# xytpai/kfunca

Hardware: AMD Instinct MI355X
Metric: bf16 GEMM TFLOP/s + causal-attn fwd+bwd tokens/s (higher is better)
Workload: dtype bf16

## Files before the change

kfunca_amd/csrc/device/attention.hip:

```cpp
#include <math.h>
#include <stdlib.h>

#include <algorithm>
#include <type_traits>

#include "common.h"

namespace kf {

typedef __attribute__((ext_vector_type(8))) __bf16 bf16x8;
typedef __attribute__((ext_vector_type(8))) _Float16 f16x8;
typedef __attribute__((ext_vector_type(4))) short s16x4;
typedef __attribute__((ext_vector_type(8))) short s16x8;
typedef __attribute__((ext_vector_type(16))) float f32x16;
typedef __attribute__((ext_vector_type(4))) float f32x4;

struct AttnArgs {
    const char *q, *k, *v, *o, *d_o;
    char *out, *dq, *dk, *dv;
    float *lse;
    const float *lse_r;
    float *delta;
    float *nlse, *ndelta;
    int64_t B, H, Sq, Skv, D;
// ... 400 lines not shown
        const int64_t kv0 = (int64_t)t * ABK;
        TL_STAMP(6)
        asm volatile("s_waitcnt vmcnt(4)" ::: "memory");
        TL_STAMP(0)
        __builtin_amdgcn_s_barrier();
        asm volatile("" ::: "memory");
        TL_STAMP(1)
        stage(t + 2, smem + ((t + 2) % SRING) * FBUF);
        TL_STAMP(2)
        const char *cur = smem + (t % SRING) * FBUF;
        const bool skip = !active || kv0 > qw + 31 || KF_MUT(1, t == 1 && qblk == nxb - 1);
        const bool diag = kv0 + ABK - 1 > qw;
        if (late && pending) s_pv<BF, DB>(smem + ((t + SRING - 1) % SRING) * FBUF + FTILE, vo, pf, o);
        pending = false;
        TL_STAMP(5)
        if (!skip) {
            if (diag) s_qk_sm<BF, true, D>(cur, qf, ko, o, pf, m_i, l_i, c, kv0, m, hl, a.defer TL_ARGS);
            else s_qk_sm<BF, false, D>(cur, qf, ko, o, pf, m_i, l_i, c, kv0, m, hl, a.defer TL_ARGS);
            TL_STAMP(4)
            if (late) pending = true;
            else s_pv<BF, DB>(cur + FTILE, vo, pf, o);
            TL_STAMP(5)
        }
    }
#if defined(KF_ATTN_TIMELINE) && KF_ATTN_TIMELINE != 2
    if (lane == 0 && g_attn_tl) {
        unsigned long long *dst = g_attn_tl + ((size_t)blockIdx.x * 2 + (pass & 1)) * 64 + wid * 8;
        for (int i = 0; i < 7; ++i) dst[i] = tl_acc[i];
        dst[7] = (unsigned long long)nt;
    }
#endif
#ifdef KF_ATTN_TIMELINE
    const unsigned long long tl_loop1 = __builtin_amdgcn_s_memtime();
#endif
    if (late && pending) s_pv<BF, DB>(smem + ((nt + SRING - 1) % SRING) * FBUF + FTILE, vo, pf, o);
    asm volatile("s_waitcnt vmcnt(0)" ::: "memory");
    __syncthreads();
    if (active) {
        a_store_rows<BF, DB>(smem + wid * 32 * OPAD, a.out + a_head(a.lo, bh, a.H) + qw * a.lo.sr, o, 1.f / l_i, a.lo.sr);
        if (a.lse && hl == 0) a.lse[bh * a.Sq + m] = (m_i * c + __builtin_amdgcn_logf(l_i)) * kLn2;
    }
    if (a.persist) __syncthreads();
#if defined(KF_ATTN_TIMELINE) && KF_ATTN_TIMELINE == 2
    if (lane == 0 && g_attn_tl) {
        unsigned long long *dst = g_attn_tl + ((size_t)blockIdx.x * 2 + (pass & 1)) * 64 + wid * 8;
        const unsigned long long tl_end = __builtin_amdgcn_s_memtime();
        dst[0] = tl_loop0 - tl_pass0, dst[1] = tl_loop1 - tl_loop0, dst[2] = tl_end - tl_loop1;
        dst[3] = dst[4] = dst[5] = dst[6] = 0;
        dst[7] = (unsigned long long)nt;
    }
#endif
  }
}

#ifndef KF_FWD_W4_INC
#define KF_FWD_W4_INC "attn_fwd_w4.inc"
#endif
#include KF_FWD_W4_INC
template <bool BF, bool SQ, bool D64 = false>
__global__ __launch_bounds__(256) void attn_fwd_w4_kernel(const AttnArgs a) {
    static_assert(!(SQ && D64), "the scaled-query form exists for head size 128 only");
    extern __shared__ __attribute__((aligned(16))) char smem[];
    const int nxb = (int)((a.Sq + FQ - 1) / FQ);
    const int nwx = a.persist ? nxb / 2 : nxb;
    const unsigned lds = (unsigned)(uintptr_t)(const __attribute__((address_space(3))) char *)smem;
    const int wid = __builtin_amdgcn_readfirstlane(threadIdx.x >> 6);
    const int dbytes = D64 ? 128 : 256;
    const unsigned kvn = (unsigned)((a.Skv - 1) * a.lk.sr + dbytes);
    const float c = a.scale_log2e, defer = a.defer;
    const int qsr = (int)a.lq.sr, kvsr = (int)a.lk.sr, osr = (int)a.lo.sr;
#pragma nounroll
    for (unsigned vwg = blockIdx.x; vwg < a.nvwg; vwg += gridDim.x) {
    int xb0;
    int64_t bh;
    a_block_map(nwx, a.nbh, a.xcd_map, xb0, bh, vwg);
    const char *kp = a.k + a_head_kv(a.lk, bh, a.H, a.G), *vp = a.v + a_head_kv(a.lv, bh, a.H, a.G);
    const char *qh = a.q + a_head(a.lq, bh, a.H);
    char *oh = a.out + a_head(a.lo, bh, a.H);
#pragma nounroll
    for (int pass = 0; pass < (a.persist ? 2 : 1); ++pass) {
        const int xb = ((pass & 1) != (a.persist_rev != 0)) ? nxb - 1 - xb0 : xb0;
        const int qblk = nxb - 1 - xb;
        const int64_t q0 = (int64_t)qblk * FQ;
        const char *qp = qh + q0 * a.lq.sr;
        char *op = oh + q0 * a.lo.sr;
        float *lsep = a.lse ? a.lse + bh * a.Sq + q0 : nullptr;
        const int T = (int)((q0 + FQ) / ABK);
        const int64_t qrows = a.Sq - q0 < FQ ? a.Sq - q0 : FQ;
        const unsigned qn = (unsigned)((qrows - 1) * a.lq.sr + dbytes), on = (unsigned)((qrows - 1) * a.lo.sr + dbytes), lsen = (unsigned)(qrows * 4);
        int mut = -1;
#ifdef KF_MUTANT
        if (a.mutant == 1 && qblk == nxb - 1) mut = 1;
#endif
#ifdef KF_FWD_W4_STAMPS
        unsigned long long *dbg = a.dbg;
        const unsigned dbgoff = (vwg * 2 + pass) * 4 * 32;
#define KF_W4_EXTRA , [dbg] "s"(dbg), [dbgoff] "s"(dbgoff)
#else
#define KF_W4_EXTRA
#endif
#define KF_W4_OPERANDS                                                                                                              \
    [qp] "s"(qp), [kp] "s"(kp), [vp] "s"(vp), [op] "s"(op), [lsep] "s"(lsep), [qsr] "s"(qsr), [kvsr] "s"(kvsr), [osr] "s"(osr), [T] "s"(T), \
        [wid] "s"(wid), [c] "s"(c), [defer] "s"(defer), [lds] "s"(lds), [mut] "s"(mut), [kvn] "s"(kvn), [qn] "s"(qn), [on] "s"(on), [lsen] "s"(lsen) KF_W4_EXTRA
        if constexpr (D64 && BF) asm volatile(KF_FWD_W4_D64_ASM_BF16 : : KF_W4_OPERANDS : KF_FWD_W4_CLOBBERS);
        else if constexpr (D64) asm volatile(KF_FWD_W4_D64_ASM_F16 : : KF_W4_OPERANDS : KF_FWD_W4_CLOBBERS);
        else if constexpr (BF && SQ) asm volatile(KF_FWD_W4_ASM_BF16_SQ : : KF_W4_OPERANDS : KF_FWD_W4_CLOBBERS);
        else if constexpr (BF) asm volatile(KF_FWD_W4_ASM_BF16 : : KF_W4_OPERANDS : KF_FWD_W4_CLOBBERS);
        else if constexpr (SQ) asm volatile(KF_FWD_W4_ASM_F16_SQ : : KF_W4_OPERANDS : KF_FWD_W4_CLOBBERS);
        else asm volatile(KF_FWD_W4_ASM_F16 : : KF_W4_OPERANDS : KF_FWD_W4_CLOBBERS);
#undef KF_W4_OPERANDS
#undef KF_W4_EXTRA
    }
    }
}

template <bool BF, int R>
__global__ __launch_bounds__(256) void attn_delta_kernel(const char *o, const char *d_o, float *delta, int64_t nrows, const float *lse, float *nlse,
                                                         float *ndelta, float rscale, AttnArgs::Lay lo, AttnArgs::Lay ldo, int64_t S, int64_t H, int nparts, int64_t Sc) {
    const int64_t row0 = (int64_t)blockIdx.x * (16 * R) + (threadIdx.x >> 4);
    const int part = threadIdx.x & 15;
    uint4 a[R], b[R];
#pragma unroll
    for (int i = 0; i < R; ++i) {
        a[i] = b[i] = uint4{0, 0, 0, 0};
        const int64_t row = row0 + 16 * i;
        const int64_t bh = row / Sc, sq = row - bh * Sc;
        if (row < nrows && sq < S && part < nparts) {
            a[i] = *(const uint4 *)(o + a_head(lo, bh, H) + sq * lo.sr + part * 16);
            b[i] = *(const uint4 *)(d_o + a_head(ldo, bh, H) + sq * ldo.sr + part * 16);
        }
    }
#pragma unroll
    for (int i = 0; i < R; ++i) {
        const int64_t row = row0 + 16 * i;
        float acc = 0.f;
        const uint32_t aw[4] = {a[i].x, a[i].y, a[i].z, a[i].w}, bw[4] = {b[i].x, b[i].y, b[i].z, b[i].w};
#pragma unroll
        for (int j = 0; j < 4; ++j) {
            float a0, a1, b0, b1;
            if constexpr (BF) {
                a0 = __uint_as_float(aw[j] << 16); a1 = __uint_as_float(aw[j] & 0xffff0000u);
                b0 = __uint_as_float(bw[j] << 16); b1 = __uint_as_float(bw[j] & 0xffff0000u);
            } else {
                a0 = f16_to_f32(f16_t{(uint16_t)(aw[j] & 0xffff)}); a1 = f16_to_f32(f16_t{(uint16_t)(aw[j] >> 16)});
                b0 = f16_to_f32(f16_t{(uint16_t)(bw[j] & 0xffff)}); b1 = f16_to_f32(f16_t{(uint16_t)(bw[j] >> 16)});
            }
            acc += a0 * b0 + a1 * b1;
        }
        for (int msk = 8; msk > 0; msk >>= 1) acc += __shfl_xor(acc, msk, 64);
        if (row < nrows && part == 0) {
            const int64_t bh = row / Sc, sq = row - bh * Sc;
            if (sq < S) {
                delta[bh * S + sq] = acc;
                if (nlse) {
                    nlse[row] = -lse[bh * S + sq] * rscale;
                    ndelta[row] = -acc;
                }
            } else if (nlse) {
                nlse[row] = 0.f;
                ndelta[row] = 0.f;
            }
        }
    }
}

template <bool BF, bool MASK, int D>
__device__ __forceinline__ void q_tile(const char *buf, const char *doslab, const typename AFrag<BF>::type (&qf)[D / 16], const int (&ko)[D / 16],
                                       const int (&vo)[D / 32][2], f32x16 (&dq)[D / 32], float c, float lse2, float dlt, int64_t kv0, int64_t m, int hl) {
    using frag_t = typename AFrag<BF>::type;
    constexpr int DB = D / 32;
    const char *vt = buf + FTILE;
#pragma unroll
    for (int sub = 0; sub < 2; ++sub) {
        f32x16 s, dp;
#pragma unroll
        for (int e = 0; e < 16; ++e) { s[e] = 0.f; dp[e] = 0.f; }
#pragma unroll
        for (int kg = 0; kg < D / 64; ++kg) {
#pragma unroll
            for (int kk = 4 * kg; kk < 4 * kg + 4; ++kk) s = a_mfma<BF>(*(const frag_t *)(buf + sub * 32 * AROW + ko[kk]), qf[kk], s);
            __builtin_amdgcn_sched_barrier(0);
        }
#pragma unroll
        for (int kg = 0; kg < D / 64; ++kg) {
#pragma unroll
            for (int kk = 4 * kg; kk < 4 * kg + 4; ++kk)
                dp = a_mfma<BF>(*(const frag_t *)(vt + sub * 32 * AROW + ko[kk]), *(const frag_t *)(doslab + ko[kk]), dp);
            __builtin_amdgcn_sched_barrier(0);
        }
#pragma unroll
        for (int e = 0; e < 16; ++e) {
            float p = __builtin_amdgcn_exp2f(__builtin_fmaf(s[e], c, -lse2));
            if (MASK && kv0 + sub * 32 + a_row(e, hl) > m) p = 0.f;
            s[e] = p * (dp[e] - dlt);
        }
        TrN<DB> ta;
        if (sub == 0) tr4_issue<0>(buf, vo, ta); else tr4_issue<32 * AROW>(buf, vo, ta);
        tr4_wait1(ta);
        { const frag_t df = a_pack<BF>(s, 0);
#pragma unroll
          for (int d = 0; d < DB; ++d) dq[d] = a_mfma<BF>(tr4_frag<BF, DB>(ta, d), df, dq[d]); }
        __builtin_amdgcn_sched_barrier(0);
        if (sub == 0) tr4_issue<16 * AROW>(buf, vo, ta); else tr4_issue<48 * AROW>(buf, vo, ta);
        tr4_wait1(ta);
        { const frag_t df = a_pack<BF>(s, 1);
#pragma unroll
          for (int d = 0; d < DB; ++d) dq[d] = a_mfma<BF>(tr4_frag<BF, DB>(ta, d), df, dq[d]); }
        __builtin_amdgcn_sched_barrier(0);
    }
}

constexpr int QSLAB = 32 * AROW;
constexpr int QLDS = FRING * FBUF + 8 * QSLAB;

template <bool BF, int D>
__global__ __launch_bounds__(FNT, 2) void attn_bwd_dq_v2_kernel(const AttnArgs a) {
    using frag_t = typename AFrag<BF>::type;
    constexpr int KS = D / 16, DB = D / 32;
    extern __shared__ __attribute__((aligned(16))) char smem[];
    const int lane = threadIdx.x & 63, wid = threadIdx.x >> 6, xl = lane & 31, hl = lane >> 5;
    int xb0;
    int64_t bh;
    const int nxb = (int)((a.Sq + FQ - 1) / FQ);
    const int nwx = a.persist ? nxb / (2 * a.persist) : nxb;
    a_block_map(nwx, a.nbh, a.xcd_map, xb0, bh);
    const char *Kg = a.k + a_head_kv(a.lk, bh, a.H, a.G);
    const char *Vg = a.v + a_head_kv(a.lv, bh, a.H, a.G);
    char *doslab = smem + FRING * FBUF + wid * QSLAB;
    int ko[KS], vo[DB][2];
#pragma unroll
    for (int kk = 0; kk < KS; ++kk) ko[kk] = a_off(xl, kk * 2 + hl);
#pragma unroll
    for (int d = 0; d < DB; ++d) {
        vo[d][0] = a_tr_lane_off(d * 32, 0);
        vo[d][1] = a_tr_lane_off(d * 32, 1);
    }
    const float c = a.scale * kLog2e;
#pragma nounroll
  for (int pass = 0; pass < (a.persist ? 2 * a.persist : 1); ++pass) {
    const int xp = xb0 + (pass >> 1) * nwx;
    const int xb = ((pass & 1) != (a.persist_rev != 0)) ? nxb - 1 - xp : xp;
    const int qblk = nxb - 1 - xb;
    const int64_t q0 = (int64_t)qblk * FQ, qw = q0 + wid * 32, m = qw + xl;
    const bool active = qw < a.Sq;

    frag_t qf[KS];
    float lse2 = 0.f, dlt = 0.f;
    if (active) {
        const char *Qg = a.q + a_head(a.lq, bh, a.H) + m * a.lq.sr;
#pragma unroll
        for (int kk = 0; kk < KS; ++kk) qf[kk] = *(const frag_t *)(Qg + (kk * 16 + 8 * hl) * 2);
        const char *dOw = a.d_o + a_head(a.ldo, bh, a.H) + qw * a.ldo.sr;
#pragma unroll
        for (int i = 0; i < 8; ++i)
            if (D == AD || ((lane + 64 * i) & 15) < D / 8) a_lst(doslab, lane + 64 * i, a_gld(dOw, lane + 64 * i, a.ldo.sr));
        lse2 = a.lse_r[bh * a.Sq + m] * kLog2e;
        dlt = a.delta[bh * a.Sq + m];
    } else {
#pragma unroll
        for (int kk = 0; kk < KS; ++kk)
#pragma unroll
            for (int j = 0; j < 8; ++j) qf[kk][j] = 0;
    }
    f32x16 dq[DB];
#pragma unroll
    for (int d = 0; d < DB; ++d)
#pragma unroll
        for (int e = 0; e < 16; ++e) dq[d][e] = 0.f;

    const int64_t q_end = q0 + FQ < a.Sq ? q0 + FQ : a.Sq;
    const int64_t kv_end = a.Skv < q_end ? a.Skv : q_end;
    const int nt = (int)((kv_end + ABK - 1) / ABK);
    auto stage = [&](int tile, char *buf) {
        const int64_t kv = (int64_t)(tile < nt ? tile : nt - 1) * ABK;
        f_stage<D>(Kg + kv * a.lk.sr, Vg + kv * a.lv.sr, buf, a.lk.sr, a.lv.sr);
    };
    asm volatile("s_waitcnt vmcnt(0) lgkmcnt(0)" ::: "memory");
    stage(0, smem);
    stage(1, smem + FBUF);
    for (int t = 0; t < nt; ++t) {
        const int64_t kv0 = (int64_t)t * ABK;
        asm volatile("s_waitcnt vmcnt(4)" ::: "memory");
        __builtin_amdgcn_s_barrier();
        asm volatile("" ::: "memory");
        stage(t + 2, smem + ((t + 2) % FRING) * FBUF);
        const char *cur = smem + (t % FRING) * FBUF;
        const bool skip = !active || kv0 > qw + 31 || KF_MUT(4, t == 0 && qblk == nxb - 1);
        const bool diag = kv0 + ABK - 1 > qw;
        if (!skip) {
            if (diag) q_tile<BF, true, D>(cur, doslab, qf, ko, vo, dq, c, lse2, dlt, kv0, m, hl);
            else q_tile<BF, false, D>(cur, doslab, qf, ko, vo, dq, c, lse2, dlt, kv0, m, hl);
        }
    }
    asm volatile("s_waitcnt vmcnt(0)" ::: "memory");
    __syncthreads();
    if (active) a_store_rows<BF, DB>(smem + wid * 32 * OPAD, a.dq + a_head(a.ldq, bh, a.H) + qw * a.ldq.sr, dq, a.scale, a.ldq.sr);
    if (a.persist) __syncthreads();
  }
}

constexpr int DQ_RING = 3;
constexpr int DQ_SLAB = 2 * DS_TILE;
constexpr int DQ_LDS = DQ_RING * FTILE + 8 * DQ_RING * DQ_SLAB;

template <bool BF, int HF, int KS, int DB>
__device__ __forceinline__ void dq_step(const char *kt, const int (&vo)[DB][2], unsigned dsb, f32x16 (&dq)[DB]) {
    s16x4 blo, bhi;
    TrN<DB> ta;
    asm volatile("ds_read_b64_tr_b16 %0, %2 offset:%c3\n\tds_read_b64_tr_b16 %1, %2 offset:%c4"
                 : "=&v"(blo), "=&v"(bhi)
                 : "v"(dsb), "n"(HF * DS_TILE + KS * 512), "n"(HF * DS_TILE + KS * 512 + 256)
                 : "memory");
    tr4_issue<(32 * HF + 16 * KS) * AROW>(kt, vo, ta);
    asm volatile("s_waitcnt lgkmcnt(0)" : "+v"(blo), "+v"(bhi) : : "memory");
    tr4_wait1(ta);
    s16x8 r;
    r[0] = blo[0]; r[1] = blo[1]; r[2] = blo[2]; r[3] = blo[3];
    r[4] = bhi[0]; r[5] = bhi[1]; r[6] = bhi[2]; r[7] = bhi[3];
    const auto b = __builtin_bit_cast(typename AFrag<BF>::type, r);
#pragma unroll
    for (int d = 0; d < DB; ++d) dq[d] = a_mfma<BF>(tr4_frag<BF, DB>(ta, d), b, dq[d]);
}

template <bool BF, int D>
__global__ __launch_bounds__(FNT, 2) void attn_bwd_dq_ds_kernel(const AttnArgs a) {
    constexpr int DB = D / 32;
    extern __shared__ __attribute__((aligned(16))) char smem[];
    const int lane = threadIdx.x & 63, wid = __builtin_amdgcn_readfirstlane(threadIdx.x >> 6);
    int xb0;
    int64_t bh;
    const int nxb = (int)((a.Sq + FQ - 1) / FQ);
    const int nwx = a.persist ? nxb / (2 * a.persist) : nxb;
    a_block_map(nwx, a.nbh, a.xcd_map, xb0, bh);
    bh += a.bh0;
    const char *Kg = a.k + a_head_kv(a.lk, bh, a.H, a.G);
    char *slab = smem + DQ_RING * FTILE + wid * DQ_RING * DQ_SLAB;
    int vo[DB][2];
#pragma unroll
    for (int d = 0; d < DB; ++d) {
        vo[d][0] = a_tr_lane_off(d * 32, 0);
        vo[d][1] = a_tr_lane_off(d * 32, 1);
    }
    const int grp = lane >> 4, qq = (lane >> 2) & 3, pp = lane & 3, h = grp >> 1;
    const unsigned smem_u = (unsigned)(uintptr_t)(const __attribute__((address_space(3))) char *)smem;
    const int sp = grp & 1;
    const unsigned ds_rd = smem_u + (unsigned)(slab - smem) + sp * 1024 + 64 * ((2 * h + (qq >> 1)) ^ (2 * sp)) + 32 * (qq & 1) + 16 * (pp & 1) + 8 * (pp >> 1);
    int ds_src[2];
#pragma unroll
    for (int pc = 0; pc < 2; ++pc) ds_src[pc] = pc * 1024 + (((lane >> 2) ^ (2 * pc)) * 4 + (lane & 3)) * 16;
    const int krow = lane >> 4, kpos = lane & 15;
#pragma nounroll
  for (int pass = 0; pass < (a.persist ? 2 * a.persist : 1); ++pass) {
    const int xp = xb0 + (pass >> 1) * nwx;
    const int xb = ((pass & 1) != (a.persist_rev != 0)) ? nxb - 1 - xp : xp;
    const int qblk = nxb - 1 - xb;
    const int64_t q0 = (int64_t)qblk * FQ, qw = q0 + wid * 32;
    const bool active = qw < a.Sq;
    const int sl = (int)(qw >> 5);
    f32x16 dq[DB];
#pragma unroll
    for (int d = 0; d < DB; ++d)
#pragma unroll
        for (int e = 0; e < 16; ++e) dq[d][e] = 0.f;
    const int64_t q_end = q0 + FQ < a.Sq ? q0 + FQ : a.Sq;
    const int64_t kv_end = a.Skv < q_end ? a.Skv : q_end;
    const int nt = (int)((kv_end + ABK - 1) / ABK);
    const char *dsg = a.ds + ((bh - a.bh0) * a.ds_pair + ds_row_base(qblk, a.ds_nkb, a.ds_tri) + wid) * DS_TILE;
    const int kwb_last = (int)(a.ds_nkb * 8 - 1);
    const int slw = qblk * 8 + wid;
    auto stage = [&](int tile, int slot) {
        const int tl = tile < nt ? tile : nt - 1;
        const int kfirst = tl * ABK, klast = (int)a.Skv - 1 - kfirst;
        const char *kg = Kg + (int64_t)kfirst * a.lk.sr;
#pragma unroll
        for (int i = 0; i < 2; ++i) {
            const int row0 = (wid * 2 + i) * 4, row = row0 + krow;
            const int chunk = kpos ^ (((row & 3) << 2) | ((row >> 2) & 3));
            const int srow = row < klast ? row : klast;
            if (D == AD || chunk < D / 8)
                __builtin_amdgcn_global_load_lds((const __attribute__((address_space(1))) void *)(kg + (int64_t)srow * a.lk.sr + chunk * 16),
                                                 (__attribute__((address_space(3))) void *)(smem + slot * FTILE + row0 * AROW), 16, 0, 0);
        }
#pragma unroll
        for (int hf = 0; hf < 2; ++hf) {
            int kwb = 2 * tl + hf;
            kwb = kwb < kwb_last ? kwb : kwb_last;
            kwb = kwb <= slw ? kwb : (slw < kwb_last ? slw : kwb_last);
            const char *tg = dsg + (int64_t)kwb * 8 * DS_TILE;
#pragma unroll
            for (int pc = 0; pc < 2; ++pc)
                __builtin_amdgcn_global_load_lds((const __attribute__((address_space(1))) void *)(tg + ds_src[pc]),
                                                 (__attribute__((address_space(3))) void *)(slab + slot * DQ_SLAB + hf * DS_TILE + pc * 1024), 16, 0, 0);
        }
    };
    stage(0, 0);
    stage(1, 1);
    for (int t = 0; t < nt; ++t) {
        asm volatile("s_waitcnt vmcnt(6)" ::: "memory");
        __builtin_amdgcn_s_barrier();
        asm volatile("" ::: "memory");
        stage(t + 2, (t + 2) % DQ_RING);
        const char *kt = smem + (t % DQ_RING) * FTILE;
        const unsigned dsb = ds_rd + (unsigned)((t % DQ_RING) * DQ_SLAB);
        if (active && 2 * t <= sl && !KF_MUT(3, t == 0 && qblk == nxb - 1)) {
            dq_step<BF, 0, 0, DB>(kt, vo, dsb, dq);
            dq_step<BF, 0, 1, DB>(kt, vo, dsb, dq);
            if (2 * t + 1 <= sl) {
                dq_step<BF, 1, 0, DB>(kt, vo, dsb, dq);
                dq_step<BF, 1, 1, DB>(kt, vo, dsb, dq);
            }
        }
    }
    asm volatile("s_waitcnt vmcnt(0)" ::: "memory");
    __syncthreads();
    if (active) a_store_rows<BF, DB>(smem + wid * 32 * OPAD, a.dq + a_head(a.ldq, bh, a.H) + qw * a.ldq.sr, dq, a.scale, a.ldq.sr,
                                     (int)(a.Sq - qw < 32 ? a.Sq - qw : 32));
    if (a.persist) __syncthreads();
  }
}

constexpr int BQS = 32;

constexpr int K4B = 128;
constexpr int K4SL = 2 * BQS * AROW + 256;
constexpr int K4PAIR = 2 * K4SL;
constexpr int K4LDS = 4 * K4PAIR;
constexpr bool K4_SPREAD = true;
static_assert(K4LDS >= 4 * 32 * OPAD, "epilogue slabs must fit");

template <int OFF>
__device__ __forceinline__ void k4_rows4(unsigned e, unsigned o, s16x8 (&f)[4]) {
    asm volatile("ds_read_b128 %0, %4 offset:%c6\n\tds_read_b128 %1, %5 offset:%c6\n\t"
                 "ds_read_b128 %2, %4 offset:%c7\n\tds_read_b128 %3, %5 offset:%c7"
                 : "=&v"(f[0]), "=&v"(f[1]), "=&v"(f[2]), "=&v"(f[3])
                 : "v"(e), "v"(o), "n"(OFF), "n"(OFF + 512)
                 : "memory");
}
template <int OFF>
__device__ __forceinline__ void k4_rowc(unsigned lr, f32x4 (&c)[4]) {
    asm volatile("ds_read_b128 %0, %4 offset:%c5\n\tds_read_b128 %1, %4 offset:%c6\n\t"
                 "ds_read_b128 %2, %4 offset:%c7\n\tds_read_b128 %3, %4 offset:%c8"
                 : "=&a"(c[0]), "=&a"(c[1]), "=&a"(c[2]), "=&a"(c[3])
                 : "v"(lr), "n"(OFF), "n"(OFF + 32), "n"(OFF + 64), "n"(OFF + 96)
                 : "memory");
}
struct K4Tr { s16x4 lo[4], hi[4]; };
template <int OFF>
__device__ __forceinline__ void k4_tr4(unsigned t0, unsigned t1, K4Tr &t) {
    asm volatile("ds_read_b64_tr_b16 %0, %8 offset:%c10\n\tds_read_b64_tr_b16 %1, %9 offset:%c10\n\t"
                 "ds_read_b64_tr_b16 %2, %8 offset:%c11\n\tds_read_b64_tr_b16 %3, %9 offset:%c11\n\t"
                 "ds_read_b64_tr_b16 %4, %8 offset:%c12\n\tds_read_b64_tr_b16 %5, %9 offset:%c12\n\t"
                 "ds_read_b64_tr_b16 %6, %8 offset:%c13\n\tds_read_b64_tr_b16 %7, %9 offset:%c13"
                 : "=&v"(t.lo[0]), "=&v"(t.hi[0]), "=&v"(t.lo[1]), "=&v"(t.hi[1]), "=&v"(t.lo[2]), "=&v"(t.hi[2]), "=&v"(t.lo[3]), "=&v"(t.hi[3])
                 : "v"(t0), "v"(t1), "n"(OFF), "n"(OFF + 512), "n"(OFF + 1024), "n"(OFF + 1536)
                 : "memory");
}
template <int N>
__device__ __forceinline__ void k4_wait4(s16x8 (&f)[4]) {
    asm volatile("s_waitcnt lgkmcnt(%c4)" : "+v"(f[0]), "+v"(f[1]), "+v"(f[2]), "+v"(f[3]) : "n"(N) : "memory");
}
template <int N>
__device__ __forceinline__ void k4_wait4c(s16x8 (&f)[4], f32x4 (&c)[4]) {
    asm volatile("s_waitcnt lgkmcnt(%c8)"
                 : "+v"(f[0]), "+v"(f[1]), "+v"(f[2]), "+v"(f[3]), "+a"(c[0]), "+a"(c[1]), "+a"(c[2]), "+a"(c[3])
                 : "n"(N)
                 : "memory");
}
template <int N>
__device__ __forceinline__ void k4_wait_tr(K4Tr &a) {
    asm volatile("s_waitcnt lgkmcnt(%c8)"
                 : "+v"(a.lo[0]), "+v"(a.hi[0]), "+v"(a.lo[1]), "+v"(a.hi[1]), "+v"(a.lo[2]), "+v"(a.hi[2]), "+v"(a.lo[3]), "+v"(a.hi[3])
                 : "n"(N)
                 : "memory");
}
template <bool BF>
__device__ __forceinline__ typename AFrag<BF>::type k4_frag(const K4Tr &t, int d) {
    s16x8 r;
    r[0] = t.lo[d][0]; r[1] = t.lo[d][1]; r[2] = t.lo[d][2]; r[3] = t.lo[d][3];
    r[4] = t.hi[d][0]; r[5] = t.hi[d][1]; r[6] = t.hi[d][2]; r[7] = t.hi[d][3];
    return __builtin_bit_cast(typename AFrag<BF>::type, r);
}
__device__ __forceinline__ f32x16 k4_acc(const f32x4 (&c)[4]) {
    f32x16 r;
#pragma unroll
    for (int g = 0; g < 4; ++g)
#pragma unroll
        for (int j = 0; j < 4; ++j) r[4 * g + j] = c[g][j];
    return r;
}

template <int OFF>
__device__ __forceinline__ void k4_rows4a(unsigned e, unsigned o, s16x8 (&f)[4]) {
    asm volatile("ds_read_b128 %0, %4 offset:%c6\n\tds_read_b128 %1, %5 offset:%c6\n\t"
                 "ds_read_b128 %2, %4 offset:%c7\n\tds_read_b128 %3, %5 offset:%c7"
                 : "=&a"(f[0]), "=&a"(f[1]), "=&a"(f[2]), "=&a"(f[3])
                 : "v"(e), "v"(o), "n"(OFF), "n"(OFF + 512)
                 : "memory");
}
template <int OFF>
__device__ __forceinline__ void k4_rowcv(unsigned lr, f32x4 (&c)[4]) {
    asm volatile("ds_read_b128 %0, %4 offset:%c5\n\tds_read_b128 %1, %4 offset:%c6\n\t"
                 "ds_read_b128 %2, %4 offset:%c7\n\tds_read_b128 %3, %4 offset:%c8"
                 : "=&v"(c[0]), "=&v"(c[1]), "=&v"(c[2]), "=&v"(c[3])
                 : "v"(lr), "n"(OFF), "n"(OFF + 32), "n"(OFF + 64), "n"(OFF + 96)
                 : "memory");
}
template <int N>
__device__ __forceinline__ void k4_wait4a_cv(s16x8 (&f)[4], f32x4 (&c)[4]) {
    asm volatile("s_waitcnt lgkmcnt(%c8)"
                 : "+a"(f[0]), "+a"(f[1]), "+a"(f[2]), "+a"(f[3]), "+v"(c[0]), "+v"(c[1]), "+v"(c[2]), "+v"(c[3])
                 : "n"(N)
                 : "memory");
}
template <int N>
__device__ __forceinline__ void k4_wait4a(s16x8 (&f)[4]) {
    asm volatile("s_waitcnt lgkmcnt(%c4)" : "+a"(f[0]), "+a"(f[1]), "+a"(f[2]), "+a"(f[3]) : "n"(N) : "memory");
}
template <int N>
__device__ __forceinline__ void k4_wait4_cv(s16x8 (&f)[4], f32x4 (&c)[4]) {
    asm volatile("s_waitcnt lgkmcnt(%c8)"
                 : "+v"(f[0]), "+v"(f[1]), "+v"(f[2]), "+v"(f[3]), "+v"(c[0]), "+v"(c[1]), "+v"(c[2]), "+v"(c[3])
                 : "n"(N)
                 : "memory");
}
template <int OFF>
__device__ __forceinline__ void k4_row1(unsigned a, s16x8 &f) { asm volatile("ds_read_b128 %0, %1 offset:%c2" : "=&v"(f) : "v"(a), "n"(OFF) : "memory"); }
template <int OFF>
__device__ __forceinline__ void k4_row1a(unsigned a, s16x8 &f) { asm volatile("ds_read_b128 %0, %1 offset:%c2" : "=&a"(f) : "v"(a), "n"(OFF) : "memory"); }
template <int OFF>
__device__ __forceinline__ void k4_rowc1(unsigned lr, f32x4 &c) { asm volatile("ds_read_b128 %0, %1 offset:%c2" : "=&v"(c) : "v"(lr), "n"(OFF) : "memory"); }
template <int OFF>
__device__ __forceinline__ void k4_trp(unsigned t0, unsigned t1, s16x4 &lo, s16x4 &hi) {
    asm volatile("ds_read_b64_tr_b16 %0, %2 offset:%c4\n\tds_read_b64_tr_b16 %1, %3 offset:%c4" : "=&v"(lo), "=&v"(hi) : "v"(t0), "v"(t1), "n"(OFF) : "memory");
}
template <bool BF, bool AA>
__device__ __forceinline__ void k4_mfma_first(f32x16 &acc, s16x8 &a, const typename AFrag<BF>::type &b, f32x16 &c) {
    if constexpr (BF) {
        if constexpr (AA) asm volatile("s_nop 1\n\tv_mfma_f32_32x32x16_bf16 %0, %1, %3, %2" : "=&v"(acc), "+a"(a), "+v"(c) : "a"(b));
        else asm volatile("s_nop 1\n\tv_mfma_f32_32x32x16_bf16 %0, %1, %3, %2" : "=&v"(acc), "+v"(a), "+v"(c) : "a"(b));
    } else {
        if constexpr (AA) asm volatile("s_nop 1\n\tv_mfma_f32_32x32x16_f16 %0, %1, %3, %2" : "=&v"(acc), "+a"(a), "+v"(c) : "a"(b));
        else asm volatile("s_nop 1\n\tv_mfma_f32_32x32x16_f16 %0, %1, %3, %2" : "=&v"(acc), "+v"(a), "+v"(c) : "a"(b));
    }
}
template <bool BF, bool AA>
__device__ __forceinline__ void k4_mfma_acc(f32x16 &acc, s16x8 &a, const typename AFrag<BF>::type &b) {
    if constexpr (BF) {
        if constexpr (AA) asm volatile("v_mfma_f32_32x32x16_bf16 %0, %1, %2, %0" : "+v"(acc), "+a"(a) : "a"(b));
        else asm volatile("v_mfma_f32_32x32x16_bf16 %0, %1, %2, %0" : "+v"(acc), "+v"(a) : "a"(b));
    } else {
        if constexpr (AA) asm volatile("v_mfma_f32_32x32x16_f16 %0, %1, %2, %0" : "+v"(acc), "+a"(a) : "a"(b));
        else asm volatile("v_mfma_f32_32x32x16_f16 %0, %1, %2, %0" : "+v"(acc), "+v"(a) : "a"(b));
    }
}
template <bool BF>
__device__ __forceinline__ void k4_mfma_first_t(f32x16 &acc, s16x8 &a, const typename AFrag<BF>::type &b, f32x16 &c, f32x16 &tag) {
    if constexpr (BF) asm volatile("s_nop 1\n\tv_mfma_f32_32x32x16_bf16 %0, %1, %4, %2\n\ts_nop 3" : "=&v"(acc), "+v"(a), "+v"(c), "+v"(tag) : "a"(b));
    else asm volatile("s_nop 1\n\tv_mfma_f32_32x32x16_f16 %0, %1, %4, %2\n\ts_nop 3" : "=&v"(acc), "+v"(a), "+v"(c), "+v"(tag) : "a"(b));
}
template <bool BF>
__device__ __forceinline__ void k4_mfma_acc_t(f32x16 &acc, s16x8 &a, const typename AFrag<BF>::type &b, f32x16 &tag) {
    if constexpr (BF) asm volatile("v_mfma_f32_32x32x16_bf16 %0, %1, %3, %0" : "+v"(acc), "+v"(a), "+v"(tag) : "a"(b));
    else asm volatile("v_mfma_f32_32x32x16_f16 %0, %1, %3, %0" : "+v"(acc), "+v"(a), "+v"(tag) : "a"(b));
}
__device__ __forceinline__ void k4_keep(s16x8 (&f)[4]) { asm volatile("" : "+v"(f[0]), "+v"(f[1]), "+v"(f[2]), "+v"(f[3])); }
__device__ __forceinline__ void k4_keep(f32x16 &c) { asm volatile("" : "+v"(c)); }

template <int OFF>
__device__ __forceinline__ void k4_tr2(unsigned t0, unsigned t1, K4Tr &t) {
    asm volatile("ds_read_b64_tr_b16 %0, %4 offset:%c6\n\tds_read_b64_tr_b16 %1, %5 offset:%c6\n\t"
                 "ds_read_b64_tr_b16 %2, %4 offset:%c7\n\tds_read_b64_tr_b16 %3, %5 offset:%c7"
                 : "=&v"(t.lo[0]), "=&v"(t.hi[0]), "=&v"(t.lo[1]), "=&v"(t.hi[1])
                 : "v"(t0), "v"(t1), "n"(OFF), "n"(OFF + 512)
                 : "memory");
}
template <int N>
__device__ __forceinline__ void k4_wait_tr2(K4Tr &a) {
    asm volatile("s_waitcnt lgkmcnt(%c4)" : "+v"(a.lo[0]), "+v"(a.hi[0]), "+v"(a.lo[1]), "+v"(a.hi[1]) : "n"(N) : "memory");
}

__device__ __forceinline__ float k4_mul(float a, float b) { return a * b; }
__device__ __forceinline__ float k4_mul_odd(float a, float b) { return __builtin_fmaf(a, b, 0.f); }
#ifdef KF_ABL_DKV_NOVALU
#define KF_ABL_EXP(x) (x)
#define KF_ABL_MUL(a, b) (b)
#define KF_ABL_MUL_ODD(a, b) (b)
#else
#define KF_ABL_EXP(x) __builtin_amdgcn_exp2f(x)
#define KF_ABL_MUL(a, b) k4_mul(a, b)
#define KF_ABL_MUL_ODD(a, b) k4_mul_odd(a, b)
#endif
template <bool BF, bool DS, int D>
__global__ __launch_bounds__(256) void attn_bwd_dkv_v4_kernel(const AttnArgs a) {
    using frag_t = typename AFrag<BF>::type;
    constexpr int KS = D / 16, DB = D / 32;
    extern __shared__ __attribute__((aligned(16))) char smem[];
    const int lane = threadIdx.x & 63, wid = __builtin_amdgcn_readfirstlane(threadIdx.x >> 6), xl = lane & 31, hl = lane >> 5;
    int xb0;
    int64_t bh;
    const int nkb = (int)(a.Skv / K4B), nwx = a.persist ? nkb / (2 * a.persist) : nkb;
    a_block_map(nwx, a.nbh, a.xcd_map, xb0, bh);
    bh += a.bh0;
    const char *Qg = a.q + a_head(a.lq, bh, a.H);
    const char *dOg = a.d_o + a_head(a.ldo, bh, a.H);
    const char *Kh = a.k + a_head_kv(a.lk, bh, a.H, a.G), *Vh = a.v + a_head_kv(a.lv, bh, a.H, a.G);
#pragma nounroll
  for (int pass = 0; pass < (a.persist ? 2 * a.persist : 1); ++pass) {
    const int xp = xb0 + (pass >> 1) * nwx;
    const int xb = ((pass & 1) != (a.persist_rev != 0)) ? nkb - 1 - xp : xp;
    const int64_t k0 = (int64_t)xb * K4B, kw = k0 + wid * 32, n = kw + xl;
#ifdef KF_ATTN_TIMELINE
    const unsigned long long tl_pass0 = __builtin_amdgcn_s_memtime();
#endif

    frag_t kf[8], vf[8];
    const float c = a.scale * kLog2e;
    {
        const char *Kg = Kh + n * a.lk.sr;
        const char *Vg = Vh + n * a.lv.sr;
#pragma unroll
        for (int kk = 0; kk < KS; ++kk) {
            kf[kk] = *(const frag_t *)(Kg + (kk * 16 + 8 * hl) * 2);
            vf[kk] = *(const frag_t *)(Vg + (kk * 16 + 8 * hl) * 2);
        }
    }
    f32x16 dk[4], dv[4];
#pragma unroll
    for (int d = 0; d < DB; ++d)
#pragma unroll
        for (int e = 0; e < 16; ++e) { dk[d][e] = 0.f; dv[d][e] = 0.f; }

    const unsigned smem_u = (unsigned)(uintptr_t)(const __attribute__((address_space(3))) char *)smem;
    const int rsw = (xl >> 2) & 3;
    const unsigned rb_e = smem_u + 2048 * (xl >> 3) + 64 * (xl & 7) + 16 * ((0 + hl) ^ rsw);
    const unsigned rb_o = smem_u + 2048 * (xl >> 3) + 64 * (xl & 7) + 16 * ((2 + hl) ^ rsw);
    const int g = lane >> 4, qq = (lane & 15) >> 2, pp = lane & 3, h = g >> 1;
    const int tslot = 2 * (g & 1) + (pp >> 1);
    const unsigned tb_0 = smem_u + 64 * (4 * h + qq) + 16 * (tslot ^ h) + 8 * (pp & 1);
    const unsigned tb_1 = smem_u + 2048 + 64 * (4 * h + qq) + 16 * (tslot ^ (h + 2)) + 8 * (pp & 1);
    const unsigned lr = smem_u + 2 * BQS * AROW + 16 * hl;

    int64_t soffq[2], soffd[2];
#pragma unroll
    for (int i = 0; i < 2; ++i) {
        const int sub = 2 * i + (lane >> 5), r = (lane >> 2) & 7, slot = lane & 3, row = 8 * wid + r;
        const int ch = (4 * sub + (slot ^ ((row >> 2) & 3))) * 16;
        soffq[i] = row * a.lq.sr + ch;
        soffd[i] = row * a.ldo.sr + ch;
    }
    const float *rcg = lane < BQS ? a.nlse + bh * a.Sqc + lane : a.ndelta + bh * a.Sqc + lane - BQS;
    const int ns = (int)(a.Sq / BQS), np = ns / 2;
    unsigned ds_lane = (unsigned)(xl * 32 + hl * 16);
    const char *ds_base = DS ? a.ds + ((bh - a.bh0) * a.ds_pair + (kw >> 5) * 8) * DS_TILE : nullptr;
    const int ds_nkb = (int)a.ds_nkb, ds_tri = a.ds_tri;
    auto stage_piece = [&](auto id_c, int pr_, int slot4) __attribute__((always_inline)) {
        constexpr int ID = decltype(id_c)::value, SL = ID / 5, K = ID % 5;
        if constexpr (D == 64 && (K == 2 || K == 3)) return;
        const int prc = pr_ < np ? pr_ : np - 1;
        const int64_t qs_ = ((int64_t)prc * 2 + SL) * BQS;
        char *buf = smem + slot4 * K4PAIR + SL * K4SL;
        if constexpr (K == 4) {
            __builtin_amdgcn_global_load_lds((const __attribute__((address_space(1))) void *)(rcg + qs_),
                                             (__attribute__((address_space(3))) void *)(buf + 2 * BQS * AROW), 4, 0, 0);
        } else {
            constexpr int i = K >> 1;
            const char *src = (K & 1) ? dOg + qs_ * a.ldo.sr + soffd[i] : Qg + qs_ * a.lq.sr + soffq[i];
            __builtin_amdgcn_global_load_lds((const __attribute__((address_space(1))) void *)src,
                                             (__attribute__((address_space(3))) void *)(buf + (K & 1) * BQS * AROW + 1024 * (2 * wid + i)), 16, 0, 0);
        }
    };
    auto stage_pair = [&](int pr_, int slot4) __attribute__((always_inline)) {
        stage_piece(std::integral_constant<int, 0>{}, pr_, slot4); stage_piece(std::integral_constant<int, 1>{}, pr_, slot4);
        stage_piece(std::integral_constant<int, 2>{}, pr_, slot4); stage_piece(std::integral_constant<int, 3>{}, pr_, slot4);
        stage_piece(std::integral_constant<int, 4>{}, pr_, slot4); stage_piece(std::integral_constant<int, 5>{}, pr_, slot4);
        stage_piece(std::integral_constant<int, 6>{}, pr_, slot4); stage_piece(std::integral_constant<int, 7>{}, pr_, slot4);
        stage_piece(std::integral_constant<int, 8>{}, pr_, slot4); stage_piece(std::integral_constant<int, 9>{}, pr_, slot4);
    };

    const int p0 = (int)(k0 / (2 * BQS));
    stage_pair(p0, 0);
    stage_pair(p0 + 1, 1);
    stage_pair(p0 + 2, 2);
    {
#pragma unroll
        for (int kk = 0; kk < KS; ++kk) asm volatile("" : "+a"(kf[kk]), "+a"(vf[kk]));
    }
    if constexpr (D == 128) asm volatile("s_waitcnt vmcnt(10)" ::: "memory");
    else asm volatile("s_waitcnt vmcnt(6)" ::: "memory");
    __builtin_amdgcn_s_barrier();
    asm volatile("" ::: "memory");

#ifdef KF_ATTN_TIMELINE
    unsigned long long tlk[10], tlk_acc[11] = {0, 0, 0, 0, 0, 0, 0, 0, 0, 0, 0}, tlk_prev = __builtin_amdgcn_s_memtime();
#endif
    s16x8 g0[4], g1[4];
    f32x4 cs[4], cp[4];
    if constexpr (D == 128) {
        k4_rowcv<0>(lr, cs);
        k4_rows4a<0>(rb_e, rb_o, g0);
        k4_rows4a<1024>(rb_e, rb_o, g1);
        k4_rowcv<128>(lr, cp);
    } else {
        k4_rowcv<0>(lr, cs);
        k4_rows4a<0>(rb_e, rb_o, g0);
        k4_rowcv<128>(lr, cp);
        k4_rows4<BQS * AROW>(rb_e, rb_o, g1);
    }

#define K4_MFMA4(ACC, FR, BOP, K0)                                                                                   \
    _Pragma("unroll") for (int kk = 0; kk < 4; ++kk) ACC = a_mfma<BF>(__builtin_bit_cast(frag_t, FR[kk]), BOP[K0 + kk], ACC);
#define K4_CVT2(DST, J, A, B)                                              \
    if constexpr (BF) { DST[J] = (__bf16)(A); DST[(J) + 1] = (__bf16)(B); } \
    else { DST[J] = (_Float16)(A); DST[(J) + 1] = (_Float16)(B); }
#define K4_CVTP(DST, J, A, B)                                              \
// ... 1520 lines not shown
```

Baseline: 7.756 million.

## Skip redundant clamped dS/K tile loads in dQ kernel pipeline tail

Splits the dQ kernel's staging loop into a steady-state phase that loads full K and dS tiles and a tail phase that issues only the loads it needs. Beyond the causal limit, the old code kept loading clamped duplicate tiles. The tail now skips those loads and adjusts the vmcnt wait depth to match the number of loads actually issued. It also sets a nontemporal cache hint on the dS loads. The added branching and per-wave variable wait counts make the code more complex and carry some risk of synchronization mistakes.

Result: no change. 7.826 million (median of 6 runs) (+0.9%).

```diff
diff --git a/kfunca_amd/csrc/device/attention.hip b/kfunca_amd/csrc/device/attention.hip
--- a/kfunca_amd/csrc/device/attention.hip
+++ b/kfunca_amd/csrc/device/attention.hip
@@ -726,6 +726,7 @@
 constexpr int DQ_RING = 3;
 constexpr int DQ_SLAB = 2 * DS_TILE;
 constexpr int DQ_LDS = DQ_RING * FTILE + 8 * DQ_RING * DQ_SLAB;
+constexpr int DQ_AUX_NT = 2;
 
 template <bool BF, int HF, int KS, int DB>
 __device__ __forceinline__ void dq_step(const char *kt, const int (&vo)[DB][2], unsigned dsb, f32x16 (&dq)[DB]) {
@@ -792,38 +793,7 @@
     const char *dsg = a.ds + ((bh - a.bh0) * a.ds_pair + ds_row_base(qblk, a.ds_nkb, a.ds_tri) + wid) * DS_TILE;
     const int kwb_last = (int)(a.ds_nkb * 8 - 1);
     const int slw = qblk * 8 + wid;
-    auto stage = [&](int tile, int slot) {
-        const int tl = tile < nt ? tile : nt - 1;
-        const int kfirst = tl * ABK, klast = (int)a.Skv - 1 - kfirst;
-        const char *kg = Kg + (int64_t)kfirst * a.lk.sr;
-#pragma unroll
-        for (int i = 0; i < 2; ++i) {
-            const int row0 = (wid * 2 + i) * 4, row = row0 + krow;
-            const int chunk = kpos ^ (((row & 3) << 2) | ((row >> 2) & 3));
-            const int srow = row < klast ? row : klast;
-            if (D == AD || chunk < D / 8)
-                __builtin_amdgcn_global_load_lds((const __attribute__((address_space(1))) void *)(kg + (int64_t)srow * a.lk.sr + chunk * 16),
-                                                 (__attribute__((address_space(3))) void *)(smem + slot * FTILE + row0 * AROW), 16, 0, 0);
-        }
-#pragma unroll
-        for (int hf = 0; hf < 2; ++hf) {
-            int kwb = 2 * tl + hf;
-            kwb = kwb < kwb_last ? kwb : kwb_last;
-            kwb = kwb <= slw ? kwb : (slw < kwb_last ? slw : kwb_last);
-            const char *tg = dsg + (int64_t)kwb * 8 * DS_TILE;
-#pragma unroll
-            for (int pc = 0; pc < 2; ++pc)
-                __builtin_amdgcn_global_load_lds((const __attribute__((address_space(1))) void *)(tg + ds_src[pc]),
-                                                 (__attribute__((address_space(3))) void *)(slab + slot * DQ_SLAB + hf * DS_TILE + pc * 1024), 16, 0, 0);
-        }
-    };
-    stage(0, 0);
-    stage(1, 1);
-    for (int t = 0; t < nt; ++t) {
-        asm volatile("s_waitcnt vmcnt(6)" ::: "memory");
-        __builtin_amdgcn_s_barrier();
-        asm volatile("" ::: "memory");
-        stage(t + 2, (t + 2) % DQ_RING);
+    auto consume = [&](int t) {
         const char *kt = smem + (t % DQ_RING) * FTILE;
         const unsigned dsb = ds_rd + (unsigned)((t % DQ_RING) * DQ_SLAB);
         if (active && 2 * t <= sl && !KF_MUT(3, t == 0 && qblk == nxb - 1)) {
@@ -834,6 +804,66 @@
                 dq_step<BF, 1, 1, DB>(kt, vo, dsb, dq);
             }
         }
+    };
+    const int kwb_lim = active ? (slw < kwb_last ? slw : kwb_last) : -1;
+    const int nfull = nt < ((kwb_lim + 1) >> 1) ? nt : ((kwb_lim + 1) >> 1);
+    auto stage_k = [&](int tile, int slot) {
+        const int kfirst = tile * ABK, klast = (int)a.Skv - 1 - kfirst;
+        const char *kg = Kg + (int64_t)kfirst * a.lk.sr;
+#pragma unroll
+        for (int i = 0; i < 2; ++i) {
+            const int row0 = (wid * 2 + i) * 4, row = row0 + krow;
+            const int chunk = kpos ^ (((row & 3) << 2) | ((row >> 2) & 3));
+            const int srow = row < klast ? row : klast;
+            if (D == AD || chunk < D / 8)
+                __builtin_amdgcn_global_load_lds((const __attribute__((address_space(1))) void *)(kg + (int64_t)srow * a.lk.sr + chunk * 16),
+                                                 (__attribute__((address_space(3))) void *)(smem + slot * FTILE + row0 * AROW), 16, 0, 0);
+        }
+    };
+    auto stage_ds = [&](int kwb, int slot) {
+        const char *tg = dsg + (int64_t)kwb * 8 * DS_TILE;
+#pragma unroll
+        for (int pc = 0; pc < 2; ++pc)
+            __builtin_amdgcn_global_load_lds((const __attribute__((address_space(1))) void *)(tg + ds_src[pc]),
+                                             (__attribute__((address_space(3))) void *)(slab + slot * DQ_SLAB + (kwb & 1) * DS_TILE + pc * 1024), 16, 0,
+                                             DQ_AUX_NT);
+    };
+    auto stage_tail = [&](int tile, int slot) -> int {
+        if (tile >= nt) return 0;
+        stage_k(tile, slot);
+        int n = 2;
+#pragma unroll
+        for (int hf = 0; hf < 2; ++hf)
+            if (2 * tile + hf <= kwb_lim) {
+                stage_ds(2 * tile + hf, slot);
+                n += 2;
+            }
+        return n;
+    };
+    int behind = 0;
+#pragma unroll
+    for (int i = 0; i < 2; ++i) behind = stage_tail(i, i);
+    int t = 0;
+    for (; t + 2 < nfull; ++t) {
+        asm volatile("s_waitcnt vmcnt(6)" ::: "memory");
+        __builtin_amdgcn_s_barrier();
+        asm volatile("" ::: "memory");
+        const int slot = (t + 2) % DQ_RING;
+        stage_k(t + 2, slot);
+        stage_ds(2 * t + 4, slot);
+        stage_ds(2 * t + 5, slot);
+        consume(t);
+    }
+    if (t > 0) behind = 6;
+    for (; t < nt; ++t) {
+        if (behind == 6) asm volatile("s_waitcnt vmcnt(6)" ::: "memory");
+        else if (behind == 4) asm volatile("s_waitcnt vmcnt(4)" ::: "memory");
+        else if (behind == 2) asm volatile("s_waitcnt vmcnt(2)" ::: "memory");
+        else asm volatile("s_waitcnt vmcnt(0)" ::: "memory");
+        __builtin_amdgcn_s_barrier();
+        asm volatile("" ::: "memory");
+        behind = stage_tail(t + 2, (t + 2) % DQ_RING);
+        consume(t);
     }
     asm volatile("s_waitcnt vmcnt(0)" ::: "memory");
     __syncthreads();
```
